# imironhead/ml_super_resolution

Measured on AMD Instinct MI355X. Metric: VDSR-20 training patches/sec (41x41, batch 256 per GPU); fwd HR megapixels/sec alongside, higher is better.
Workload: dtype f32; 1 GPU; BASELINE configs[2]: VDSR 20-layer 3x3x64 residual, RGB, batch 256x41x41 per GPU, fwd+bwd+TF-Adam, random-init weights; global_batch=256, patch=41, parallelism=dp1

## Files before the change

### include/srx.h

```cpp
#ifndef SRX_H_
#define SRX_H_

#include <stddef.h>
#include <stdint.h>

#ifdef __cplusplus
extern "C" {
#endif

typedef void* srx_stream_t;

typedef enum {
    SRX_OK = 0,
    SRX_ERR_BAD_ARG = -1,
    SRX_ERR_UNSUPPORTED = -2,
    SRX_ERR_WORKSPACE = -3,
    SRX_ERR_LAUNCH = -4,
    SRX_ERR_ALIGN = -5
} srx_status;

typedef enum { SRX_PAD_SAME = 0, SRX_PAD_VALID = 1 } srx_pad_mode;

typedef enum {
    SRX_ACT_NONE = 0,
// ... 33 lines not shown

int srx_set_chain_fixed(int on);

int srx_conv2d_precision_supported(const srx_conv_desc* d, int op);

size_t srx_conv2d_workspace_bytes(const srx_conv_desc* d, int op);

int srx_conv2d_fwd(const srx_conv_desc* d, const float* x, const float* w, const float* bias,
                   const float* skip, float* y, void* ws, size_t ws_bytes, srx_stream_t stream);

int srx_conv2d_bwd_data(const srx_conv_desc* d, const float* dpre, const float* w,
                        const float* x_in, int in_act, float* dx_out, void* ws, size_t ws_bytes,
                        srx_stream_t stream);

int srx_conv2d_bwd_data_acc(const srx_conv_desc* d, const float* dpre, const float* w, const float* dx_acc,
                            float* dx_out, void* ws, size_t ws_bytes, srx_stream_t stream);

int srx_conv2d_bwd_filter(const srx_conv_desc* d, const float* x, const float* dpre, float* dw,
                          float* dbias, const float* w_for_decay, float wd_scale, void* ws,
                          size_t ws_bytes, srx_stream_t stream);

int srx_conv2d_bwd_filter_partials(const srx_conv_desc* d, const float* x, const float* dpre, void* ws,
                                   size_t ws_bytes, int* n_partials, srx_stream_t stream);
int srx_conv2d_bwd_filter_reduce(const srx_conv_desc* d, const void* ws, int n_partials, float* dw,
                                 float* dbias, const float* w_for_decay, float wd_scale,
                                 srx_stream_t stream);

int srx_conv2d_bwd_filter_batch(const srx_conv_desc* d, int n_layers, const float* const* x, const float* const* dpre,
                                float* const* dw, float* const* dbias, const float* const* w_for_decay, float wd_scale,
                                void* ws, size_t ws_bytes, srx_stream_t stream);
size_t srx_conv2d_bwd_filter_batch_workspace_bytes(const srx_conv_desc* d, int n_layers);
int srx_conv2d_bwd_filter_batch_plan(const srx_conv_desc* d, int n_layers, int* wgs_per_layer, int* grid);
int srx_set_wgrad_batch(int on);

int srx_act_bwd(const float* dy, const float* y, float* dpre, size_t numel, int act,
                srx_stream_t stream);

int srx_depth_to_space(const float* in, float* out, int N, int H, int W, int C, int r,
                       srx_stream_t stream);

int srx_stream_copy(const void* in, void* out, size_t bytes, srx_stream_t stream);

int srx_espcn_forward(const float* x, const float* w1, const float* b1, const float* w2, const float* b2,
                      const float* w3, const float* b3, float* hr, int N, int H, int W, int r,
                      srx_stream_t stream);
int srx_espcn_forward_keep(const float* x, const float* w1, const float* b1, const float* w2, const float* b2,
                           const float* w3, const float* b3, float* t1, float* t2, float* y, int N, int H, int W, int r,
                           srx_stream_t stream);

int srx_srcnn_forward(const float* x, const float* w1, const float* b1, const float* w2, const float* b2,
                      const float* w3, const float* b3, float* y, int N, int H, int W, srx_stream_t stream);

int srx_space_to_depth(const float* in, float* out, int N, int H, int W, int C, int r,
                       srx_stream_t stream);

int srx_mse_fwd_bwd(const float* pred, const float* target, size_t numel, float inv_numel,
                    float* loss_out, int accumulate, float* dpred, void* scratch,
                    srx_stream_t stream);

int srx_l2_loss(const float* w, const float* mask, size_t numel, float scale, float* loss_out,
                int accumulate, void* scratch, srx_stream_t stream);

size_t srx_reduce_scratch_bytes(void);

int srx_adam_tf_step(float* w, const float* g, float* m, float* v, size_t numel, float lr,
                     float beta1, float beta2, float eps, int64_t t, float grad_scale,
// ... 287 lines not shown
```

### ml_super_resolution_amd/_lib.py

```python
import ctypes
import os

_HERE = os.path.dirname(os.path.abspath(__file__))
LIB_PATH = os.path.join(_HERE, 'libsrx.so')

SRX_OK = 0
PAD_SAME, PAD_VALID = 0, 1
ACT_NONE, ACT_RELU, ACT_TANH, ACT_LRELU, ACT_SIGMOID = 0, 1, 2, 3, 4
OP_FWD, OP_BWD_DATA, OP_BWD_FILTER = 0, 1, 2
PRECISION_FP32, PRECISION_BF16X3 = 0, 1
PRECISION_BY_NAME = {'highest': PRECISION_FP32, 'high': PRECISION_BF16X3}

ACT_BY_NAME = {None: ACT_NONE, 'none': ACT_NONE, 'relu': ACT_RELU, 'tanh': ACT_TANH,
               'lrelu': ACT_LRELU, 'leaky_relu': ACT_LRELU, 'sigmoid': ACT_SIGMOID}
PAD_BY_NAME = {'same': PAD_SAME, 'valid': PAD_VALID}

EXPORTS = [
    'srx_version', 'srx_last_error', 'srx_set_conv_path', 'srx_set_wgrad_path', 'srx_set_chain', 'srx_set_chain_fixed', 'srx_conv_chain', 'srx_conv_chain_supported', 'srx_conv2d_precision_supported', 'srx_conv2d_workspace_bytes', 'srx_conv2d_fwd',
    'srx_conv2d_bwd_data', 'srx_conv2d_bwd_filter', 'srx_conv2d_bwd_filter_partials', 'srx_conv2d_bwd_filter_reduce',
    'srx_conv2d_bwd_filter_batch', 'srx_conv2d_bwd_filter_batch_workspace_bytes', 'srx_conv2d_bwd_filter_batch_plan', 'srx_set_wgrad_batch', 'srx_act_bwd', 'srx_depth_to_space',
    'srx_space_to_depth', 'srx_stream_copy', 'srx_mse_fwd_bwd', 'srx_l2_loss', 'srx_reduce_scratch_bytes',
    'srx_adam_tf_step', 'srx_adam_tf_step_dev', 'srx_momentum_clip_step', 'srx_rownorm_loss_fwd_bwd', 'srx_psnr', 'srx_ssim', 'srx_ssim_scratch_bytes', 'srx_saturate_u8', 'srx_affine', 'srx_u8_to_unit_float', 'srx_gaussian_blur', 'srx_resize_bilinear',
    'srx_upsample_nearest', 'srx_upsample_nearest_bwd', 'srx_add_relu_grad',
    'srx_conv2d_bwd_data_acc', 'srx_conv3x3_blocked', 'srx_conv3x3_blocked_bwd_filter_workspace_bytes', 'srx_conv3x3_blocked_bwd_filter',
    'srx_conv3x3_blocked_ex', 'srx_conv3x3_blocked_bwd_filter_ex_workspace_bytes', 'srx_conv3x3_blocked_bwd_filter_ex',
    'srx_espcn_forward', 'srx_espcn_forward_keep', 'srx_debug_poison_lds', 'srx_srcnn_forward', 'srx_maxpool2x2', 'srx_maxpool2x2_bwd', 'srx_maxpool2x2_bwd_masked', 'srx_subsample2', 'srx_subsample2_bwd',
    'srx_channel_blocks_to_nhwc', 'srx_nhwc_to_channel_blocks', 'srx_channel_normalize', 'srx_channel_normalize_bwd',
    'srx_extract_patches16', 'srx_texture_gram', 'srx_texture_gram_bwd', 'srx_pil_resample_ksize', 'srx_pil_resample_coeffs', 'srx_resample_u8', 'srx_u8_to_pm1', 'srx_log_loss', 'srx_vgg_preprocess', 'srx_add_scaled', 'srx_resize_bicubic_tf', 'srx_column_sums', 'srx_gemm_workspace_bytes', 'srx_gemm',
    'srx_feature_mosaic_u8', 'srx_summary_panel_bytes', 'srx_summary_panel_range_bytes', 'srx_summary_panel_u8', 'srx_summary_panel_range',
    'srx_vdsr_patch_table_check', 'srx_vdsr_patch_pairs',
    'srx_espcn_patch_table_check', 'srx_espcn_patch_pairs',
    'srx_espcn_eval_table_check', 'srx_espcn_eval_tiles', 'srx_espcn_eval_pairs',
    'srx_vdsr_eval_table_check', 'srx_vdsr_eval_tiles', 'srx_vdsr_eval_footprint', 'srx_vdsr_eval_pairs',
    'srx_enet_pairs_table_words', 'srx_enet_pairs_tables', 'srx_enet_patch_table_check', 'srx_enet_patch_pairs',
    'srx_enet_eval_coeff_words', 'srx_enet_eval_coeffs', 'srx_enet_eval_table_check', 'srx_enet_eval_tiles', 'srx_enet_eval_footprint',
    'srx_enet_eval_pairs',
    'srx_image_scores_scratch_bytes', 'srx_image_scores_plan', 'srx_image_scores_lds_bytes', 'srx_image_scores',
    'srx_srcnn_pairs_band', 'srx_srcnn_pairs_lds_bytes', 'srx_srcnn_patch_table_check', 'srx_srcnn_patch_pairs',
    'srx_srcnn_eval_table_check', 'srx_srcnn_eval_tiles', 'srx_srcnn_eval_footprint', 'srx_srcnn_eval_pairs',
]


class SrxError(RuntimeError):
    pass


class ConvDesc(ctypes.Structure):
    _fields_ = [(n, ctypes.c_int32) for n in
                ('N', 'H', 'W', 'Cin', 'Cout', 'KH', 'KW', 'stride', 'pad_mode', 'act',
                 'post_add_relu', 'precision', 'subpixel_r')]


class PatchSrc(ctypes.Structure):
# ... 64 lines not shown
    global _lib
    if _lib is not None:
        return _lib
    if not os.path.exists(LIB_PATH):
        raise SrxError('libsrx.so not found at %s -- build it with `make -C %s` (or '
                       '__graft_entry__.build()); there is no CPU fallback' %
                       (LIB_PATH, os.path.join(_HERE, 'csrc')))
    import torch
    L = ctypes.CDLL(LIB_PATH)
    vp, sz, i, f = ctypes.c_void_p, ctypes.c_size_t, ctypes.c_int, ctypes.c_float
    dp = ctypes.POINTER(ConvDesc)
    L.srx_version.restype = ctypes.c_char_p
    L.srx_last_error.restype = ctypes.c_char_p
    L.srx_set_conv_path.argtypes = [i]
    L.srx_set_wgrad_path.argtypes = [i]
    L.srx_set_chain.argtypes = [i]
    L.srx_set_chain_fixed.argtypes = [i]
    L.srx_conv_chain_supported.argtypes = [dp, i, i]
    L.srx_conv_chain.argtypes = [dp, i, i, i, vp, vp, vp, vp, vp, vp]
    L.srx_conv2d_precision_supported.argtypes = [dp, i]
    L.srx_conv2d_workspace_bytes.argtypes = [dp, i]
    L.srx_conv2d_workspace_bytes.restype = sz
    L.srx_reduce_scratch_bytes.restype = sz
    L.srx_conv2d_fwd.argtypes = [dp, vp, vp, vp, vp, vp, vp, sz, vp]
    L.srx_conv2d_bwd_data.argtypes = [dp, vp, vp, vp, i, vp, vp, sz, vp]
    L.srx_conv2d_bwd_filter.argtypes = [dp, vp, vp, vp, vp, vp, f, vp, sz, vp]
    L.srx_conv2d_bwd_filter_partials.argtypes = [dp, vp, vp, vp, sz, ctypes.POINTER(ctypes.c_int), vp]
    L.srx_conv2d_bwd_filter_reduce.argtypes = [dp, vp, i, vp, vp, vp, f, vp]
    L.srx_conv2d_bwd_filter_batch.argtypes = [dp, i, vp, vp, vp, vp, vp, f, vp, sz, vp]
    L.srx_conv2d_bwd_filter_batch_workspace_bytes.argtypes = [dp, i]
    L.srx_conv2d_bwd_filter_batch_workspace_bytes.restype = sz
    L.srx_conv2d_bwd_filter_batch_plan.argtypes = [dp, i, ctypes.POINTER(ctypes.c_int), ctypes.POINTER(ctypes.c_int)]
    L.srx_set_wgrad_batch.argtypes = [i]
    L.srx_act_bwd.argtypes = [vp, vp, vp, sz, i, vp]
    L.srx_depth_to_space.argtypes = [vp, vp, i, i, i, i, i, vp]
    L.srx_space_to_depth.argtypes = [vp, vp, i, i, i, i, i, vp]
    L.srx_stream_copy.argtypes = [vp, vp, sz, vp]
    L.srx_mse_fwd_bwd.argtypes = [vp, vp, sz, f, vp, i, vp, vp, vp]
    L.srx_l2_loss.argtypes = [vp, vp, sz, f, vp, i, vp, vp]
    L.srx_adam_tf_step.argtypes = [vp, vp, vp, vp, sz, f, f, f, f, ctypes.c_int64, f, vp]
    L.srx_adam_tf_step_dev.argtypes = [vp, vp, vp, vp, sz, vp, f, f, f, f, vp]
    L.srx_momentum_clip_step.argtypes = [vp, vp, vp, sz, f, f, f, f, vp]
    L.srx_rownorm_loss_fwd_bwd.argtypes = [vp, vp, sz, sz, vp, vp, vp, vp]
    L.srx_psnr.argtypes = [vp, vp, vp, i, sz, f, vp]
    L.srx_ssim.argtypes = [vp, vp, vp, i, i, i, i, f, vp, vp]
    L.srx_ssim_scratch_bytes.argtypes = [i]
    L.srx_ssim_scratch_bytes.restype = sz
    sp, ip = ctypes.POINTER(ScoresDesc), ctypes.POINTER(ctypes.c_int)
    L.srx_image_scores_scratch_bytes.argtypes = [sp]
    L.srx_image_scores_scratch_bytes.restype = sz
    L.srx_image_scores_plan.argtypes = [sp, ip, ip, ip, ip]
    L.srx_image_scores_lds_bytes.argtypes = [sp]
    L.srx_image_scores_lds_bytes.restype = sz
    L.srx_image_scores.argtypes = [sp, vp, vp, vp, vp, vp]
    L.srx_saturate_u8.argtypes = [vp, vp, sz, vp]
    L.srx_feature_mosaic_u8.argtypes = [vp, vp, i, i, i, vp]
    L.srx_summary_panel_bytes.argtypes = [vp, i, i, i, i]
    L.srx_summary_panel_bytes.restype = sz
    L.srx_summary_panel_range_bytes.restype = sz
    L.srx_summary_panel_u8.argtypes = [vp, i, i, i, i, vp, vp, vp]
    L.srx_summary_panel_range.argtypes = [vp, i, i, i, i, vp, vp]
    L.srx_vdsr_patch_table_check.argtypes = [vp, i, i, sz]
    L.srx_vdsr_patch_pairs.argtypes = [vp, vp, i, i, vp, vp, vp]
    L.srx_espcn_patch_table_check.argtypes = [vp, i, i, i, sz]
    L.srx_espcn_patch_pairs.argtypes = [vp, vp, i, i, i, vp, vp, vp]
    L.srx_espcn_eval_table_check.argtypes = [vp, i, i, sz, sz]
# ... 82 lines not shown
```

### ml_super_resolution_amd/csrc/conv_narrow.hip

```cpp
#include "launchers.h"
namespace srx {
typedef float f32x3 __attribute__((ext_vector_type(3)));
typedef unsigned u32x3v __attribute__((ext_vector_type(3)));

template <int CTRL>
__device__ __forceinline__ float dpp_add(float v) {
    const int moved = __builtin_amdgcn_update_dpp(0, __float_as_int(v), CTRL, 0xf, 0xf, false);
    return v + __int_as_float(moved);
}

struct PixWalk {
    int n, oh, ow;
    __device__ __forceinline__ void init(unsigned p, int OH, int OW) {
        const unsigned t = p / (unsigned)OW;
        ow = (int)(p - t * (unsigned)OW);
        n = (int)(t / (unsigned)OH);
        oh = (int)(t - (unsigned)n * (unsigned)OH);
    }
    __device__ __forceinline__ void step16(int OH, int OW) { step(16, OH, OW); }
    __device__ __forceinline__ void step(int d, int OH, int OW) {
        ow += d;
        while (ow >= OW) {
            ow -= OW;
            oh += 1;
// ... 157 lines not shown
                idx = tc * CW + 4 * l + e;
            }
            part[idx] = r;
        } else {
            const int b = i - TAPS * 4 * CN;
            if constexpr (NOUT) {
                if (l == 0) part[wn + b] = r;
            } else {
                part[wn + 4 * l + b] = r;
            }
        }
    }
}

bool launch_wgrad_narrow(const ConvKey& k, const WgradArgs& a, int grid, hipStream_t s, hipError_t* err) {
    if (k.kh != 3 || k.kw != 3) return false;
    const bool nout = a.Cin == 64 && a.Cout == 3, nin = a.Cin == 3 && a.Cout == 64, nin32 = a.Cin == 3 && a.Cout == 32;
    if (!nout && !nin && !nin32) return false;
    const long total = (long)a.N * a.OH * a.OW;
    if (total >= (1L << 31) - 4096 || (long)a.N * a.H * a.W * 64 * 4 >= (1L << 31) - 4096 || total * 64 * 4 >= (1L << 31) - 4096)
        return false;
    const long ppi = nin32 ? 32 : 16;
    const int iters = (int)((total + ppi * grid - 1) / (ppi * grid));
    if (nout)
        hipLaunchKernelGGL((wgrad_narrow_kernel<3, 3, true>), dim3(grid), dim3(256), 0, s, a, total, iters);
    else if (nin)
        hipLaunchKernelGGL((wgrad_narrow_kernel<3, 3, false>), dim3(grid), dim3(256), 0, s, a, total, iters);
    else
        hipLaunchKernelGGL((wgrad_narrow_kernel<3, 3, false, 32>), dim3(grid), dim3(256), 0, s, a, total, iters);
    *err = hipGetLastError();
    return true;
}

bool launch_conv_narrow(const ConvKey& k, const ConvArgs& a, hipStream_t s, hipError_t* err) {
    if (k.wt || a.Cout != 3 || a.mask) return false;
    if ((long)a.N * a.H * a.W * a.Cin * 4 >= (1L << 31) - 4096) return false;
    const long total = (long)a.N * a.OH * a.OW;
    int iters = 16;
    while (iters > 1 && total / (16L * iters) < 2048) iters >>= 1;
    const long blocks = (total + 16L * iters - 1) / (16L * iters);
    if (total >= (1L << 31) - 4096) return false;
    if (k.kh == 3 && k.kw == 3 && a.Cin == 64) {
        hipLaunchKernelGGL((conv_narrow_kernel<3, 3, 64, 3>), dim3((unsigned)blocks), dim3(256), 0, s, a, total, iters);
    } else {
        return false;
    }
    *err = hipGetLastError();
    return true;
}
}
```

### ml_super_resolution_amd/csrc/launchers.h

```cpp
#pragma once
#include "conv_kernels.hip.h"
#include "lds_launch.h"

namespace srx {

struct ConvKey {
    int kh, kw, cinp, nch;
    bool wt;
};

bool launch_conv_k3c64(const ConvKey& k, const ConvArgs& a, int grid, size_t lds, hipStream_t s, hipError_t* err);
bool launch_conv_k3c32(const ConvKey& k, const ConvArgs& a, int grid, size_t lds, hipStream_t s, hipError_t* err);
bool launch_conv_c4(const ConvKey& k, const ConvArgs& a, int grid, size_t lds, hipStream_t s, hipError_t* err);
bool launch_conv_misc(const ConvKey& k, const ConvArgs& a, int grid, size_t lds, hipStream_t s, hipError_t* err);
bool launch_pipe_k3c64(const ConvKey& k, const ConvArgs& a, int grid, size_t lds, hipStream_t s, hipError_t* err);
bool launch_pipe_other(const ConvKey& k, const ConvArgs& a, int grid, size_t lds, hipStream_t s, hipError_t* err);
bool launch_wgrad_narrow(const ConvKey& k, const WgradArgs& a, int grid, hipStream_t s, hipError_t* err);
bool launch_conv_narrow(const ConvKey& k, const ConvArgs& a, hipStream_t s, hipError_t* err);
bool launch_conv_1x1(const ConvKey& k, const ConvArgs& a, long min_pixels, hipStream_t s, hipError_t* err);
bool launch_conv_rows3x3(const ConvKey& k, const ConvArgs& a, long min_pixels, hipStream_t s, hipError_t* err);
bool launch_conv_pack3(const ConvKey& k, const ConvArgs& a, long min_pixels, hipStream_t s, hipError_t* err);
bool launch_conv_kwrows(const ConvKey& k, const ConvArgs& a, long min_pixels, hipStream_t s, hipError_t* err);
bool launch_pipe_strip(const ConvKey& k, const ConvArgs& a, int grid, size_t lds, hipStream_t s, hipError_t* err);
bool launch_conv_generic(const ConvKey& k, const ConvArgs& a, int grid, size_t lds, hipStream_t s, hipError_t* err);
bool launch_wgrad(const ConvKey& k, const WgradArgs& a, int grid, size_t lds, hipStream_t s, hipError_t* err);
bool launch_wgrad_generic(const ConvKey& k, const WgradArgs& a, int grid, size_t lds, hipStream_t s, hipError_t* err);
bool launch_wgrad_lin(const ConvKey& k, const WgradArgs& a, int grid, size_t lds, hipStream_t s, hipError_t* err);
bool launch_wgrad_lin_pack3(const ConvKey& k, const WgradArgs& a, int grid, size_t lds, hipStream_t s, hipError_t* err);
bool launch_wgrad_lin_strip(const ConvKey& k, const WgradArgs& a, int grid, size_t lds, hipStream_t s, hipError_t* err);
bool launch_wgrad_pipe(const ConvKey& k, const WgradArgs& a, int grid, size_t lds, hipStream_t s, hipError_t* err);
bool launch_wgrad_kwcols(const ConvKey& k, const WgradArgs& a, int max_partials, long min_pixels, int* n_partials, hipStream_t s, hipError_t* err);
bool launch_wgrad_1x1(const ConvKey& k, const WgradArgs& a, int max_partials, int* n_partials, hipStream_t s, hipError_t* err);
bool launch_wgrad_rows_full(const ConvKey& k, const WgradArgs& a, int grid, size_t lds, hipStream_t s, hipError_t* err);
bool launch_wgrad_rows_strip(const ConvKey& k, const WgradArgs& a, int grid, size_t lds, hipStream_t s, hipError_t* err);
bool launch_wgrad_lin_pairs(const ConvKey& k, const WgradPairs& q, int grid, int pairs, bool strips, size_t lds, hipStream_t s, hipError_t* err);

__attribute__((weak)) hipError_t launch_conv_chain(bool wt, bool aux, bool fixed, const ConvArgs& a, const ChainPtrs& c, int grid, size_t lds, hipStream_t s);

__attribute__((weak)) hipError_t launch_wgrad_rows_batch(const WgradArgs& a, const WgradBatchPtrs& c, int wpl, int layers, size_t lds, hipStream_t s);
__attribute__((weak)) hipError_t launch_wgrad_batch_reduce(const float* part, int wpl, int layers, int stride, int wn, int cout,
                                                           const WgradBatchOut& o, float wd, hipStream_t s);

hipError_t launch_reduce_partials(const float* part, int G, int stride, int wn, int cout, float* dw, float* dbias,
                                  const float* w, float wd, hipStream_t s);
hipError_t launch_reduce_partials_pairs(const float* part, int G, int stride, int wn, int cout, float* dw, float* dbias,
                                        int pairs, int cob, hipStream_t s);

#define SRX_LAUNCH(...) launch_with_lds<__VA_ARGS__>(dim3(grid), dim3(256), lds, s, a)

#define SRX_CONV_CASE(KH, KW, CINP, NCH, WT, MINW)                                                        \
    if (k.kh == KH && k.kw == KW && k.cinp == CINP && k.nch == NCH && k.wt == WT) {                       \
        if (a.skip || a.mask)                                                                             \
            *err = SRX_LAUNCH(conv_mfma_kernel<KH, KW, CINP, NCH, WT, MINW, true>);                       \
        else                                                                                              \
            *err = SRX_LAUNCH(conv_mfma_kernel<KH, KW, CINP, NCH, WT, MINW, false>);                      \
        return true;                                                                                      \
    }
#define SRX_PIPE_CASE_FWD(KH, KW, CINP, NCH)                                                              \
    if (k.kh == KH && k.kw == KW && k.cinp == CINP && k.nch == NCH && !k.wt) {                            \
        if (a.skip)                                                                                       \
            *err = SRX_LAUNCH(conv_pipe_kernel<KH, KW, CINP, NCH, false, 2>);                             \
        else                                                                                              \
            *err = SRX_LAUNCH(conv_pipe_kernel<KH, KW, CINP, NCH, false, 0>);                             \
        return true;                                                                                      \
    }
#define SRX_PIPE_CASE_DGRAD(KH, KW, CINP, NCH)                                                            \
    if (k.kh == KH && k.kw == KW && k.cinp == CINP && k.nch == NCH && k.wt) {                             \
        if (a.mask)                                                                                       \
            *err = SRX_LAUNCH(conv_pipe_kernel<KH, KW, CINP, NCH, true, 1>);                              \
        else                                                                                              \
            *err = SRX_LAUNCH(conv_pipe_kernel<KH, KW, CINP, NCH, true, 0>);                              \
        return true;                                                                                      \
    }
#define SRX_PIPE_STRIP_CASE(KH, KW, CINP, NCH)                                                            \
// ... 50 lines not shown
```

### ml_super_resolution_amd/csrc/srx_api.hip

```cpp
#include <math.h>
#include <stdarg.h>
#include <atomic>
#include <stdio.h>
#include <stdlib.h>
#include <string.h>

#include "../../include/srx.h"
#include "elementwise.h"
#include "launchers.h"
#include "bf16x3.h"
#include "image_scores.h"

using namespace srx;

namespace {

thread_local char g_err[512] = "";

struct Knobs {
    int pipe_default, narrow, wgrad_lin, wgrad_pipe, wgrad_pipe_strip, wgrad_rows_full, wgrad_1x1, wgrad_pack3, kwrows_min_pixels, big_route_min_pixels, strip_d2s, conv_1x1_min_pixels, pack3_dgrad;
    int chain, chain_fixed, wgrad_batch;
    unsigned long long* trace;
    int dbg;
};
int env_int(const char* name, int dflt) { const char* e = getenv(name); return e ? atoi(e) : dflt; }
Knobs read_knobs() {
    Knobs k;
    k.pipe_default = env_int("SRX_PIPE", 1);
    k.narrow = env_int("SRX_NARROW", 1);
    k.wgrad_lin = env_int("SRX_WGRAD_LIN", 1);
    k.wgrad_pipe = env_int("SRX_WGRAD_PIPE", 1);
    k.wgrad_pipe_strip = env_int("SRX_WGRAD_PIPE_STRIP", 1);
    k.kwrows_min_pixels = env_int("SRX_KWROWS_MIN_PIXELS", 4096);
    k.big_route_min_pixels = env_int("SRX_BIG_ROUTE_MIN_PIXELS", 60000);
    k.conv_1x1_min_pixels = env_int("SRX_CONV_1X1_MIN_PIXELS", 100000);
    k.pack3_dgrad = env_int("SRX_PACK3_DGRAD", 1);
    k.strip_d2s = env_int("SRX_STRIP_D2S", 1);
    k.wgrad_rows_full = env_int("SRX_WGRAD_ROWS_FULL", 1);
    k.wgrad_1x1 = env_int("SRX_WGRAD_1X1", 1);
    k.wgrad_pack3 = env_int("SRX_WGRAD_PACK3", 1);
    k.chain = env_int("SRX_CHAIN", 1);
    k.chain_fixed = env_int("SRX_CHAIN_FIXED", 1);
    k.wgrad_batch = env_int("SRX_WGRAD_BATCH", 1);
    k.trace = nullptr;
    k.dbg = 0;
#ifdef SRX_TRACE
    { const char* tp = getenv("SRX_TRACE_PTR"); k.trace = tp ? (unsigned long long*)strtoull(tp, nullptr, 0) : nullptr; }
    k.dbg = env_int("SRX_DBG", 0);
#endif
    return k;
}
const Knobs& knobs() { static const Knobs k = read_knobs(); return k; }

template <int (*Dflt)()>
struct Toggle {
    std::atomic<int> v{-1};
    int get() const { const int x = v.load(std::memory_order_relaxed); return x < 0 ? Dflt() : x; }
    int set(int x) { const int old = v.exchange(x, std::memory_order_relaxed); return old < 0 ? Dflt() : old; }
};
inline int on_off(int on) { return on < 0 ? -1 : (on ? 1 : 0); }
inline int pipe_default() { return knobs().pipe_default; }
inline int chain_default() { return knobs().chain ? 1 : 0; }
inline int chain_fixed_default() { return knobs().chain_fixed ? 1 : 0; }
inline int wgrad_batch_default() { return knobs().wgrad_batch ? 1 : 0; }
inline int wgrad_path_default() { return !knobs().wgrad_lin ? 0 : ((knobs().wgrad_pipe || knobs().wgrad_pipe_strip) ? 2 : 1); }
Toggle<pipe_default> g_use_pipe;
Toggle<chain_default> g_chain;
Toggle<chain_fixed_default> g_chain_fixed;
Toggle<wgrad_batch_default> g_wgrad_batch;
Toggle<wgrad_path_default> g_wgrad_path;
int use_pipe() { return g_use_pipe.get(); }
int wgrad_path() { return g_wgrad_path.get(); }

int cu_count() {
    static std::atomic<int> cached[64];
    int dev = 0;
    if (hipGetDevice(&dev) != hipSuccess || dev < 0 || dev >= 64) { (void)hipGetLastError(); return 256; }
    int n = cached[dev].load(std::memory_order_relaxed);
    if (n > 0) return n;
    if (hipDeviceGetAttribute(&n, hipDeviceAttributeMultiprocessorCount, dev) != hipSuccess || n <= 0) {
        (void)hipGetLastError();
        n = 256;
    }
    if (n > 256) n = 256;
    cached[dev].store(n, std::memory_order_relaxed);
    return n;
}

int fail(int code, const char* fmt, ...) {
    va_list ap;
    va_start(ap, fmt);
    vsnprintf(g_err, sizeof(g_err), fmt, ap);
    va_end(ap);
    return code;
}
int launch_status(hipError_t err, const char* what) {
    return err == hipSuccess ? SRX_OK : fail(SRX_ERR_LAUNCH, "%s: %s", what, hipGetErrorString(err));
}
}
namespace srx {
int set_error(int code, const char* fmt, ...) {
    va_list ap;
// ... 613 lines not shown
    if (kn.narrow && !s2 && launch_wgrad_narrow(k, a, p.grid, s, &err)) return taken(p.grid);
    if (wgrad_rows_strip_ok(d, lp, wpath) && launch_wgrad_rows_strip(k, a, pgrid, 2 * lin_lds, s, &err)) return taken(pgrid);
    if (kn.wgrad_pack3 && lin_ok && lin_lds <= 80 * 1024 && d->Cin == 3 && launch_wgrad_lin_pack3(k, a, p.grid, lin_lds, s, &err)) return taken(p.grid);
    if (wgrad_lin_strip_ok(d, lp, wpath) && launch_wgrad_lin_strip(k, a, p.grid, lin_lds, s, &err)) return taken(p.grid);
    if (lin_ok && lin_lds <= 80 * 1024 && launch_wgrad_lin(k, a, p.grid, lin_lds, s, &err)) return taken(p.grid);
    if (launch_wgrad(k, a, p.grid, wg_lds, s, &err)) return taken(p.grid);
    if (wg_lds <= 80 * 1024 && launch_wgrad_generic(k, a, p.grid, wg_lds, s, &err)) return taken(p.grid);
    return fail(SRX_ERR_UNSUPPORTED, "no wgrad instance for %dx%d, Cin<=%d, Cout chunks %d%s", d->KH, d->KW, p.cinp,
                p.nch, s2 ? " at stride 2" : "");
}

int srx_conv2d_bwd_filter_reduce(const srx_conv_desc* d, const void* ws, int n_partials, float* dw, float* dbias,
                                 const float* w_for_decay, float wd_scale, srx_stream_t stream) {
    int rc = check_desc(d);
    if (rc) return rc;
    if (!ws || !dw) return fail(SRX_ERR_BAD_ARG, "null tensor pointer");
    if (d->precision == SRX_PRECISION_BF16X3 && (rc = bf16x3_supported(d, SRX_OP_BWD_FILTER)) != SRX_OK) return rc;
    if (n_partials <= 0 || n_partials > kMaxGridLimit) return fail(SRX_ERR_BAD_ARG, "bad partial count %d", n_partials);
    const size_t wn = (size_t)d->KH * d->KW * d->Cin * d->Cout;
    return launch_status(launch_reduce_partials((const float*)ws, n_partials, (int)part_stride(d), (int)wn, d->Cout, dw, dbias,
                                                w_for_decay, wd_scale, (hipStream_t)stream), "reduce launch failed");
}

int srx_conv2d_bwd_filter(const srx_conv_desc* d, const float* x, const float* dpre, float* dw, float* dbias,
                          const float* w_for_decay, float wd_scale, void* ws, size_t ws_bytes, srx_stream_t stream) {
    if (!dw) return fail(SRX_ERR_BAD_ARG, "null tensor pointer");
    int n = 0;
    const int rc = srx_conv2d_bwd_filter_partials(d, x, dpre, ws, ws_bytes, &n, stream);
    if (rc) return rc;
    return srx_conv2d_bwd_filter_reduce(d, ws, n, dw, dbias, w_for_decay, wd_scale, stream);
}

namespace {
int wgrad_batch_plan(const srx_conv_desc* d, int layers, WgradArgs* a, int* wpl, int* grid, size_t* lds) {
    int rc = check_desc(d);
    if (rc) return rc;
    if (!g_wgrad_batch.get()) return fail(SRX_ERR_UNSUPPORTED, "bwd_filter_batch: switched off (srx_set_wgrad_batch / SRX_WGRAD_BATCH)");
    if (!launch_wgrad_rows_batch || !launch_wgrad_batch_reduce) return fail(SRX_ERR_UNSUPPORTED, "bwd_filter_batch: this build has no batch kernels");
    if (layers < 2 || layers > kChainMax) return fail(SRX_ERR_UNSUPPORTED, "bwd_filter_batch: %d layers (2..%d)", layers, kChainMax);
    if (d->precision != SRX_PRECISION_FP32) return fail(SRX_ERR_UNSUPPORTED, "bwd_filter_batch: precision %d (exact fp32 only)", d->precision);
    if (d->KH != 3 || d->KW != 3 || d->Cin != 64 || d->Cout != 64 || d->stride != 1 || d->pad_mode != SRX_PAD_SAME)
        return fail(SRX_ERR_UNSUPPORTED, "bwd_filter_batch: only 3x3 64->64 stride-1 SAME layers");
    if (d->W != 41) return fail(SRX_ERR_UNSUPPORTED, "bwd_filter_batch: W %d (only 41-pixel rows: wgrad_rows_full_kernel's shape)", d->W);
    const int wpath = wgrad_path();
    if (!wgrad_rows_full_switches(wpath))
        return fail(SRX_ERR_UNSUPPORTED, "bwd_filter_batch: the filter-gradient path is not wgrad_rows_full_kernel's (srx_set_wgrad_path)");
    LayerPlan lp;
    if ((rc = plan_layer(d, SRX_OP_BWD_FILTER, true, true, &lp)) != SRX_OK) return rc;
    if (!wgrad_rows_full_ok(d, lp, wpath)) return fail(SRX_ERR_UNSUPPORTED, "bwd_filter_batch: the shape is not on wgrad_rows_full_kernel's route");
    const long rows = (long)d->N * lp.OH;
    long w = pipe_grid() / layers;
    if (w > rows) w = rows;
    if (w < 1) return fail(SRX_ERR_UNSUPPORTED, "bwd_filter_batch: %d layers on a grid of %d", layers, pipe_grid());
    *wpl = (int)w;
    *grid = pipe_grid();
    fill_wgrad_args(a, d, lp);
    *lds = set_wgrad_rows_full_tile(a);
    return SRX_OK;
}
}

int srx_set_wgrad_batch(int on) { return g_wgrad_batch.set(on_off(on)); }

int srx_conv2d_bwd_filter_batch_plan(const srx_conv_desc* d, int n_layers, int* wgs_per_layer, int* grid) {
    WgradArgs a;
    int wpl = 0, g = 0;
// ... 416 lines not shown
```

### ml_super_resolution_amd/engine.py

```python
import contextlib
import gc
import math
import os

import torch

from . import ops
from .param_pool import ParamPool


@contextlib.contextmanager
def capture_graph(g):
    gc.collect()
    was_enabled = gc.isenabled()
    gc.disable()
    try:
        with torch.cuda.graph(g):
            yield
    finally:
        if was_enabled:
            gc.enable()


class LayerSpec(object):
# ... 170 lines not shown
                if ops.bwd_filter_batch_plan(acts[i].shape, s.kernel_shape, j - i, s.padding)[0] > 0:
                    best = (i, j - 1)
            i = max(j, i + 1)
        return best

    def loss_and_backward(self, target, numel_global=None):
        if self._acts is None:
            raise RuntimeError('forward(keep=True) must run before loss_and_backward')
        acts = self._acts
        y = acts[-1]
        last = len(self.specs) - 1
        inv = 1.0 / (y.numel() if numel_global is None else numel_global)
        if self.loss_kind == 'rownorm':
            row_len = y.shape[1] * y.shape[2]
            dy = ops.rownorm_loss_fwd_bwd(y, target, row_len, self.loss, dpred=self._buf(('dy', 0), y.shape),
                                          norms=self._buf(('rownorms',), (y.numel() // row_len,)))
        else:
            dy = self._buf(('dy', 0), y.shape)
            ops.mse_fwd_bwd(y, target, self.loss, inv_numel=inv, accumulate=False, dpred=dy)
        if self.weight_decay:
            self.add_regulariser_loss()
        if self.specs[last].act is not None:
            dpre = ops.act_bwd(dy, y, self.specs[last].act, out=self._buf(('dpre_last',), y.shape))
        else:
            dpre = dy
        prec = self.layer_precision
        need = max(ops.bwd_filter_workspace_bytes(acts[i].shape, s.kernel_shape, s.padding, precision=prec[i])
                   for i, s in enumerate(self.specs))
        batch = self._wgrad_batch(acts)
        if batch is not None:
            b_lo, b_hi = batch
            need = max(need, ops.bwd_filter_batch_workspace_bytes(acts[b_lo].shape, self.specs[b_lo].kernel_shape, b_hi - b_lo + 1,
                                                                  self.specs[b_lo].padding))
        if self._ws is None or self._ws.numel() * 4 < need:
            self._step_graphs.clear()
            self._ws = torch.empty((need + 3) // 4, dtype=torch.float32, device=self.device)
        chain = self._dgrad_chain(acts)
        in_batch = lambda k: batch is not None and batch[0] <= k <= batch[1]
        dpres = {}

        def wgrad(i, dpre_i):
            s = self.specs[i]
            if not in_batch(i):
                ops.conv2d_bwd_filter(acts[i], dpre_i, s.kernel_shape, s.padding,
                                      w_for_decay=self.kernel(i) if self.weight_decay else None,
                                      wd_scale=self.weight_decay, dw=self.kernel(i, self.grads),
                                      dbias=self.bias(i, self.grads), workspace=self._ws, precision=prec[i])
                return
            dpres[i] = dpre_i
            if i == batch[0]:
                ks = list(range(batch[0], batch[1] + 1))
                ops.conv2d_bwd_filter_batch([acts[k] for k in ks], [dpres[k] for k in ks], [self.kernel(k, self.grads) for k in ks],
                                            [self.bias(k, self.grads) for k in ks],
                                            [self.kernel(k) for k in ks] if self.weight_decay else None, self.weight_decay,
                                            s.padding, workspace=self._ws)

        for i in range(last, -1, -1):
            s = self.specs[i]
            if chain is not None and chain[0] <= i <= chain[1]:
                lo, hi = chain
                if i == hi:
                    outs = [self._buf(('dpre_chain', k - 1), acts[k].shape) for k in range(hi, lo - 1, -1)]
                    ops.conv2d_bwd_data_chain([dpre] + outs[:-1], [self.kernel(k) for k in range(hi, lo - 1, -1)],
                                              [acts[k] for k in range(hi, lo - 1, -1)], outs, acts[hi].shape, s.padding,
                                              in_act=self.specs[hi - 1].act)
                    cdpres = {hi: dpre}
                    for k in range(hi, lo - 1, -1):
                        cdpres[k - 1] = outs[hi - k]
                wgrad(i, cdpres[i])
                if i == lo:
                    dpre = cdpres[lo - 1]
                continue
            wgrad(i, dpre)
            if i > 0:
                prev_act = self.specs[i - 1].act
                out = (self._buf(('dpre_chain', i - 1), acts[i].shape) if in_batch(i - 1)
                       else self._buf(('dx', i % 3, acts[i].shape[3]), acts[i].shape))
                dpre = ops.conv2d_bwd_data(dpre, self.kernel(i), acts[i].shape, s.padding,
                                           x_in=acts[i] if prev_act is not None else None, in_act=prev_act, out=out,
                                           precision=prec[i])
        if self.grad_hook is not None:
            self.grad_hook(self.grads)
        return self.loss

    def add_regulariser_loss(self):
        if self._decay_mask is None:
            self._decay_mask = torch.zeros_like(self.params)
            for i in range(len(self.specs)):
                self.kernel(i, self._decay_mask).fill_(1.0)
        ops.l2_loss(self.params, self.weight_decay, self.loss, accumulate=True, mask=self._decay_mask)

    def train_step_replay(self, x, target, lr, beta1=0.9, beta2=0.999, eps=1e-8, momentum=None, gradient_cap=0.01):
        def optimizer_launch():
            if momentum is None:
                self.adam_launch_dev(beta1, beta2, eps)
            else:
                ops.momentum_clip_step(self.params, self.grads, self.opt_m, lr, momentum, gradient_cap / lr)

        def eager(xx, tt):
            self.forward(xx, keep=True)
            self.loss_and_backward(tt)
            if momentum is None:
                self.adam_step_dev(lr, beta1, beta2, eps)
            else:
                self.momentum_clip_step(lr, momentum, gradient_cap)
            return self.loss
        if not self.use_step_graph or self.grad_hook is not None or self.device.type != 'cuda':
            return eager(x, target)
        if self.step_graph_max_pixels is not None and x.shape[0] * x.shape[1] * x.shape[2] > self.step_graph_max_pixels:
            return eager(x, target)
# ... 108 lines not shown
```

### ml_super_resolution_amd/ops.py

```python
import ctypes
import os

import numpy as np
import torch

from . import _lib
from ._lib import ACT_BY_NAME, PAD_BY_NAME, ConvDesc, check
from ._lib import lib as _load_lib

_POISON_LDS = os.environ.get('SRX_POISON_LDS', '0') == '1'


def lib():
    L = _load_lib()
    if _POISON_LDS and torch.cuda.is_available():
        L.srx_debug_poison_lds(_stream())
    return L



def _stream():
    return ctypes.c_void_p(torch.cuda.current_stream().cuda_stream)


# ... 177 lines not shown
    return wpl.value, grid.value


def bwd_filter_batch_workspace_bytes(x_shape, w_shape, n_layers, padding='same', stride=1, precision='highest'):
    d = conv_desc(x_shape, w_shape, padding, stride=stride, precision=precision)
    return _load_lib().srx_conv2d_bwd_filter_batch_workspace_bytes(ctypes.byref(d), int(n_layers))


def conv2d_bwd_filter_batch(xs, dpres, dws, dbiases=None, w_for_decay=None, wd_scale=0.0, padding='same', workspace=None,
                            stride=1, precision='highest'):
    L = len(xs)
    if not (len(dpres) == len(dws) == L) or (dbiases is not None and len(dbiases) != L) or (w_for_decay is not None and len(w_for_decay) != L):
        raise ValueError('conv2d_bwd_filter_batch: the per-layer lists differ in length')
    for l in range(L):
        _chk(xs[l], 'x'); _chk(dpres[l], 'dpre'); _chk(dws[l], 'dw')
        _chk(None if dbiases is None else dbiases[l], 'dbias'); _chk(None if w_for_decay is None else w_for_decay[l], 'w_for_decay')
    d = conv_desc(xs[0].shape, dws[0].shape, padding, stride=stride, precision=precision)
    for l in range(L):
        if tuple(xs[l].shape) != tuple(xs[0].shape) or tuple(dpres[l].shape) != tuple(out_shape(d)) or tuple(dws[l].shape) != tuple(dws[0].shape):
            raise ValueError('conv2d_bwd_filter_batch: layer %d does not have the shape of layer 0' % l)
    if workspace is None:
        need = _load_lib().srx_conv2d_bwd_filter_batch_workspace_bytes(ctypes.byref(d), L)
        workspace = torch.empty((max(need, 16) + 3) // 4, dtype=torch.float32, device=xs[0].device)
    _chk(workspace, 'workspace')
    check(lib().srx_conv2d_bwd_filter_batch(ctypes.byref(d), L, _ptr_array(xs), _ptr_array(dpres), _ptr_array(dws),
                                            None if dbiases is None else _ptr_array(dbiases),
                                            None if w_for_decay is None else _ptr_array(w_for_decay), float(wd_scale),
                                            _ptr(workspace), workspace.numel() * 4, _stream()), 'srx_conv2d_bwd_filter_batch')
    return dws, dbiases


def set_wgrad_batch(on):
    return lib().srx_set_wgrad_batch(int(on))


def act_bwd(dy, y, act, out=None):
    _chk(dy, 'dy'); _chk(y, 'y')
    out = out if out is not None else torch.empty_like(dy)
    check(lib().srx_act_bwd(_ptr(dy), _ptr(y), _ptr(out), dy.numel(), ACT_BY_NAME[act], _stream()), 'srx_act_bwd')
    return out


def depth_to_space(x, r, out=None):
    _chk(x, 'x')
    N, H, W, D = x.shape
    if D % (r * r):
        raise ValueError('depth %d not divisible by r*r=%d' % (D, r * r))
    C = D // (r * r)
    out = out if out is not None else torch.empty((N, H * r, W * r, C), dtype=torch.float32, device=x.device)
    check(lib().srx_depth_to_space(_ptr(x), _ptr(out), N, H, W, C, r, _stream()), 'srx_depth_to_space')
    return out


def espcn_forward(x, params, r, out=None):
    _chk(x, 'x')
    for k, b in params:
        _chk(k, 'kernel'); _chk(b, 'bias')
    (w1, b1), (w2, b2), (w3, b3) = params
    N, H, W, C = x.shape
    if C != 3 or tuple(w1.shape) != (5, 5, 3, 64) or tuple(w2.shape) != (3, 3, 64, 32) or tuple(w3.shape) != (3, 3, 32, 3 * r * r):
        raise ValueError('espcn_forward: shapes do not describe ESPCN 5-3-3 with scaling factor %d' % r)
    out = out if out is not None else torch.empty((N, H * r, W * r, 3), dtype=torch.float32, device=x.device)
    check(lib().srx_espcn_forward(_ptr(x), _ptr(w1), _ptr(b1), _ptr(w2), _ptr(b2), _ptr(w3), _ptr(b3), _ptr(out),
                                  N, H, W, int(r), _stream()), 'srx_espcn_forward')
    return out

# ... 1095 lines not shown
```

Baseline: 20310 patches/s.

## Fuse data and filter gradients for the final 64->3 conv layer

Adds a fused backward kernel for the last 3x3 64->3 conv. A single pass reads x and dpre once and computes the input gradient (with ReLU masking), the weight-gradient partials and the bias partials, followed by a separate reduce. It replaces separate wgrad and dgrad launches that each re-read the same tensors. The engine enables it by default when the layer fits the supported shape, which adds a new code path with its own workspace sizing.

```diff
diff --git a/include/srx.h b/include/srx.h
--- a/include/srx.h
+++ b/include/srx.h
@@ -89,6 +89,13 @@
 size_t srx_conv2d_bwd_filter_batch_workspace_bytes(const srx_conv_desc* d, int n_layers);
 int srx_conv2d_bwd_filter_batch_plan(const srx_conv_desc* d, int n_layers, int* wgs_per_layer, int* grid);
 int srx_set_wgrad_batch(int on);
+
+int srx_conv2d_bwd_out3(const srx_conv_desc* d, const float* x, const float* dpre, const float* w, int in_act, float* dx,
+                        float* dw, float* dbias, const float* w_for_decay, float wd_scale, void* ws, size_t ws_bytes,
+                        srx_stream_t stream);
+size_t srx_conv2d_bwd_out3_workspace_bytes(const srx_conv_desc* d);
+int srx_conv2d_bwd_out3_plan(const srx_conv_desc* d, int in_act, int* grid, int* iters);
+int srx_set_bwd_out3(int on);
 
 int srx_act_bwd(const float* dy, const float* y, float* dpre, size_t numel, int act,
                 srx_stream_t stream);
diff --git a/ml_super_resolution_amd/_lib.py b/ml_super_resolution_amd/_lib.py
--- a/ml_super_resolution_amd/_lib.py
+++ b/ml_super_resolution_amd/_lib.py
@@ -18,7 +18,8 @@
 EXPORTS = [
     'srx_version', 'srx_last_error', 'srx_set_conv_path', 'srx_set_wgrad_path', 'srx_set_chain', 'srx_set_chain_fixed', 'srx_conv_chain', 'srx_conv_chain_supported', 'srx_conv2d_precision_supported', 'srx_conv2d_workspace_bytes', 'srx_conv2d_fwd',
     'srx_conv2d_bwd_data', 'srx_conv2d_bwd_filter', 'srx_conv2d_bwd_filter_partials', 'srx_conv2d_bwd_filter_reduce',
-    'srx_conv2d_bwd_filter_batch', 'srx_conv2d_bwd_filter_batch_workspace_bytes', 'srx_conv2d_bwd_filter_batch_plan', 'srx_set_wgrad_batch', 'srx_act_bwd', 'srx_depth_to_space',
+    'srx_conv2d_bwd_filter_batch', 'srx_conv2d_bwd_filter_batch_workspace_bytes', 'srx_conv2d_bwd_filter_batch_plan', 'srx_set_wgrad_batch',
+    'srx_conv2d_bwd_out3', 'srx_conv2d_bwd_out3_workspace_bytes', 'srx_conv2d_bwd_out3_plan', 'srx_set_bwd_out3', 'srx_act_bwd', 'srx_depth_to_space',
     'srx_space_to_depth', 'srx_stream_copy', 'srx_mse_fwd_bwd', 'srx_l2_loss', 'srx_reduce_scratch_bytes',
     'srx_adam_tf_step', 'srx_adam_tf_step_dev', 'srx_momentum_clip_step', 'srx_rownorm_loss_fwd_bwd', 'srx_psnr', 'srx_ssim', 'srx_ssim_scratch_bytes', 'srx_saturate_u8', 'srx_affine', 'srx_u8_to_unit_float', 'srx_gaussian_blur', 'srx_resize_bilinear',
     'srx_upsample_nearest', 'srx_upsample_nearest_bwd', 'srx_add_relu_grad',
@@ -149,6 +150,11 @@
     L.srx_conv2d_bwd_filter_batch_workspace_bytes.restype = sz
     L.srx_conv2d_bwd_filter_batch_plan.argtypes = [dp, i, ctypes.POINTER(ctypes.c_int), ctypes.POINTER(ctypes.c_int)]
     L.srx_set_wgrad_batch.argtypes = [i]
+    L.srx_conv2d_bwd_out3.argtypes = [dp, vp, vp, vp, i, vp, vp, vp, vp, f, vp, sz, vp]
+    L.srx_conv2d_bwd_out3_workspace_bytes.argtypes = [dp]
+    L.srx_conv2d_bwd_out3_workspace_bytes.restype = sz
+    L.srx_conv2d_bwd_out3_plan.argtypes = [dp, i, ctypes.POINTER(ctypes.c_int), ctypes.POINTER(ctypes.c_int)]
+    L.srx_set_bwd_out3.argtypes = [i]
     L.srx_act_bwd.argtypes = [vp, vp, vp, sz, i, vp]
     L.srx_depth_to_space.argtypes = [vp, vp, i, i, i, i, i, vp]
     L.srx_space_to_depth.argtypes = [vp, vp, i, i, i, i, i, vp]
diff --git a/ml_super_resolution_amd/csrc/conv_narrow.hip b/ml_super_resolution_amd/csrc/conv_narrow.hip
--- a/ml_super_resolution_amd/csrc/conv_narrow.hip
+++ b/ml_super_resolution_amd/csrc/conv_narrow.hip
@@ -213,6 +213,110 @@
     return true;
 }
 
+__global__ __launch_bounds__(256, 2) void bwd_out3_kernel(const Out3Args a, long total_px, int iters) {
+    constexpr int TAPS = 9, CN = 3, CW = 64;
+    constexpr int NV = TAPS * 4 * CN + CN;
+    __shared__ float sm[4 * NV * 16];
+    const int c4 = threadIdx.x & 15;
+    const int sub = threadIdx.x >> 4;
+    const int wave = threadIdx.x >> 6;
+    for (int i = threadIdx.x; i < TAPS * CN * CW; i += 256) {
+        const int e = i & 3, l = (i >> 2) & 15, jc = i >> 6, c = jc % CN, j = jc / CN;
+        sm[i] = a.w[((TAPS - 1 - j) * CW + 4 * l + e) * CN + c];
+    }
+    __syncthreads();
+    f32x2 acc[TAPS * CN * 2];
+    float db[CN];
+#pragma unroll
+    for (int i = 0; i < TAPS * CN * 2; ++i) acc[i] = f32x2{0.0f, 0.0f};
+#pragma unroll
+    for (int c = 0; c < CN; ++c) db[c] = 0.0f;
+    const int xbytes = a.N * a.H * a.W * CW * 4;
+    const __amdgpu_buffer_rsrc_t xrs = __builtin_amdgcn_make_buffer_rsrc(const_cast<float*>(a.x), 0, xbytes, 0x00020000);
+    const __amdgpu_buffer_rsrc_t drs = __builtin_amdgcn_make_buffer_rsrc(const_cast<float*>(a.dpre), 0, a.N * a.H * a.W * CN * 4, 0x00020000);
+    const __amdgpu_buffer_rsrc_t yrs = __builtin_amdgcn_make_buffer_rsrc(a.dx, 0, xbytes, 0x00020000);
+    const unsigned p0 = blockIdx.x * (unsigned)iters * 16u + sub;
+    const auto wide_off = [&](unsigned p) { return p < (unsigned)total_px ? (int)((p * CW + 4 * c4) * 4) : kOobOffset; };
+    PixWalk q;
+    q.init(p0 < (unsigned)total_px ? p0 : 0u, a.H, a.W);
+    const bool nomask = !a.relu_mask;
+    f32x4 xr[3];
+    f32x3 dr[3][TAPS];
+    xr[0] = __builtin_bit_cast(f32x4, __builtin_amdgcn_raw_buffer_load_b128(xrs, wide_off(p0), 0, 0));
+    xr[1] = __builtin_bit_cast(f32x4, __builtin_amdgcn_raw_buffer_load_b128(xrs, wide_off(p0 + 16u), 0, 0));
+    {
+        int off[TAPS];
+        tap_offsets<3, 3>(off, q, p0 < (unsigned)total_px, a.H, a.W, 1, 1, CN * 4, 0);
+#pragma unroll
+        for (int j = 0; j < TAPS; ++j) dr[0][j] = __builtin_bit_cast(f32x3, __builtin_amdgcn_raw_buffer_load_b96(drs, off[j], 0, 0));
+        q.step16(a.H, a.W);
+    }
+    typedef const volatile __attribute__((address_space(3))) f32x4* LdsFilter;
+    const LdsFilter wl = (LdsFilter)sm + c4;
+    for (int it = 0; it < iters; it += 3) {
+#pragma unroll
+        for (int s = 0; s < 3; ++s) {
+            if (it + s >= iters) break;
+            const unsigned p = p0 + (unsigned)(it + s) * 16u;
+            xr[(s + 2) % 3] = __builtin_bit_cast(f32x4, __builtin_amdgcn_raw_buffer_load_b128(xrs, wide_off(p + 32u), 0, 0));
+            int off[TAPS];
+            tap_offsets<3, 3>(off, q, p + 16u < (unsigned)total_px, a.H, a.W, 1, 1, CN * 4, 0);
+#pragma unroll
+            for (int j = 0; j < TAPS; ++j)
+                dr[(s + 1) % 3][j] = __builtin_bit_cast(f32x3, __builtin_amdgcn_raw_buffer_load_b96(drs, off[j], 0, 0));
+            q.step16(a.H, a.W);
+            const f32x4 xv = xr[s];
+            const f32x2 xp[2] = {f32x2{xv[0], xv[1]}, f32x2{xv[2], xv[3]}};
+            f32x2 dxp[2] = {f32x2{0.0f, 0.0f}, f32x2{0.0f, 0.0f}};
+#pragma unroll
+            for (int j = 0; j < TAPS; ++j)
+#pragma unroll
+                for (int c = 0; c < CN; ++c) {
+                    const float d = dr[s][j][c];
+                    const f32x2 dd = {d, d};
+                    const f32x4 w4 = wl[(j * CN + c) * 16];
+#pragma unroll
+                    for (int h = 0; h < 2; ++h) {
+                        acc[(j * CN + c) * 2 + h] = __builtin_elementwise_fma(xp[h], dd, acc[(j * CN + c) * 2 + h]);
+                        dxp[h] = __builtin_elementwise_fma(f32x2{w4[2 * h], w4[2 * h + 1]}, dd, dxp[h]);
+                    }
+                }
+#pragma unroll
+            for (int c = 0; c < CN; ++c) db[c] += dr[s][TAPS / 2][c];
+            f32x4 dx = {dxp[0][0], dxp[0][1], dxp[1][0], dxp[1][1]};
+#pragma unroll
+            for (int e = 0; e < 4; ++e) dx[e] = (xv[e] > 0.0f || nomask) ? dx[e] : 0.0f * dx[e];
+            __builtin_amdgcn_raw_buffer_store_b128(__builtin_bit_cast(u32x4v, dx), yrs, wide_off(p), 0, 0);
+        }
+    }
+    __syncthreads();
+#pragma unroll
+    for (int i = 0; i < NV; ++i) {
+        float r = i < NV - CN ? acc[i >> 1][i & 1] : db[i < NV - CN ? 0 : i - (NV - CN)];
+        r += __shfl_xor(r, 16);
+        r += __shfl_xor(r, 32);
+        if ((sub & 3) == 0) sm[(wave * NV + i) * 16 + c4] = r;
+    }
+    __syncthreads();
+    float* part = a.part + (size_t)blockIdx.x * a.part_stride;
+    for (int t = threadIdx.x; t < NV * 16; t += 256) {
+        const int i = t >> 4, l = t & 15;
+        const float r = (sm[(0 * NV + i) * 16 + l] + sm[(1 * NV + i) * 16 + l]) + (sm[(2 * NV + i) * 16 + l] + sm[(3 * NV + i) * 16 + l]);
+        if (i < NV - CN) {
+            const int e = i & 3, jc = i >> 2, c = jc % CN, j = jc / CN;
+            part[((TAPS - 1 - j) * CW + 4 * l + e) * CN + c] = r;
+        } else if (l == 0) {
+            part[TAPS * CW * CN + i - (NV - CN)] = r;
+        }
+    }
+}
+
+hipError_t launch_bwd_out3(const Out3Args& a, int grid, int iters, hipStream_t s) {
+    const long total = (long)a.N * a.H * a.W;
+    hipLaunchKernelGGL(bwd_out3_kernel, dim3(grid), dim3(256), 0, s, a, total, iters);
+    return hipGetLastError();
+}
+
 bool launch_conv_narrow(const ConvKey& k, const ConvArgs& a, hipStream_t s, hipError_t* err) {
     if (k.wt || a.Cout != 3 || a.mask) return false;
     if ((long)a.N * a.H * a.W * a.Cin * 4 >= (1L << 31) - 4096) return false;
diff --git a/ml_super_resolution_amd/csrc/launchers.h b/ml_super_resolution_amd/csrc/launchers.h
--- a/ml_super_resolution_amd/csrc/launchers.h
+++ b/ml_super_resolution_amd/csrc/launchers.h
@@ -40,6 +40,18 @@
 __attribute__((weak)) hipError_t launch_wgrad_rows_batch(const WgradArgs& a, const WgradBatchPtrs& c, int wpl, int layers, size_t lds, hipStream_t s);
 __attribute__((weak)) hipError_t launch_wgrad_batch_reduce(const float* part, int wpl, int layers, int stride, int wn, int cout,
                                                            const WgradBatchOut& o, float wd, hipStream_t s);
+
+struct Out3Args {
+    const float* x;
+    const float* dpre;
+    const float* w;
+    float* dx;
+    float* part;
+    int part_stride;
+    int N, H, W;
+    int relu_mask;
+};
+__attribute__((weak)) hipError_t launch_bwd_out3(const Out3Args& a, int grid, int iters, hipStream_t s);
 
 hipError_t launch_reduce_partials(const float* part, int G, int stride, int wn, int cout, float* dw, float* dbias,
                                   const float* w, float wd, hipStream_t s);
diff --git a/ml_super_resolution_amd/csrc/srx_api.hip b/ml_super_resolution_amd/csrc/srx_api.hip
--- a/ml_super_resolution_amd/csrc/srx_api.hip
+++ b/ml_super_resolution_amd/csrc/srx_api.hip
@@ -19,7 +19,7 @@
 
 struct Knobs {
     int pipe_default, narrow, wgrad_lin, wgrad_pipe, wgrad_pipe_strip, wgrad_rows_full, wgrad_1x1, wgrad_pack3, kwrows_min_pixels, big_route_min_pixels, strip_d2s, conv_1x1_min_pixels, pack3_dgrad;
-    int chain, chain_fixed, wgrad_batch;
+    int chain, chain_fixed, wgrad_batch, bwd_out3;
     unsigned long long* trace;
     int dbg;
 };
@@ -42,6 +42,7 @@
     k.chain = env_int("SRX_CHAIN", 1);
     k.chain_fixed = env_int("SRX_CHAIN_FIXED", 1);
     k.wgrad_batch = env_int("SRX_WGRAD_BATCH", 1);
+    k.bwd_out3 = env_int("SRX_BWD_OUT3", 1);
     k.trace = nullptr;
     k.dbg = 0;
 #ifdef SRX_TRACE
@@ -63,11 +64,13 @@
 inline int chain_default() { return knobs().chain ? 1 : 0; }
 inline int chain_fixed_default() { return knobs().chain_fixed ? 1 : 0; }
 inline int wgrad_batch_default() { return knobs().wgrad_batch ? 1 : 0; }
+inline int bwd_out3_default() { return (knobs().narrow && knobs().bwd_out3) ? 1 : 0; }
 inline int wgrad_path_default() { return !knobs().wgrad_lin ? 0 : ((knobs().wgrad_pipe || knobs().wgrad_pipe_strip) ? 2 : 1); }
 Toggle<pipe_default> g_use_pipe;
 Toggle<chain_default> g_chain;
 Toggle<chain_fixed_default> g_chain_fixed;
 Toggle<wgrad_batch_default> g_wgrad_batch;
+Toggle<bwd_out3_default> g_bwd_out3;
 Toggle<wgrad_path_default> g_wgrad_path;
 int use_pipe() { return g_use_pipe.get(); }
 int wgrad_path() { return g_wgrad_path.get(); }
@@ -747,6 +750,66 @@
 }
 
 namespace {
+int bwd_out3_plan(const srx_conv_desc* d, int in_act, int* grid, int* iters) {
+    int rc = check_desc(d);
+    if (rc) return rc;
+    if (!g_bwd_out3.get()) return fail(SRX_ERR_UNSUPPORTED, "bwd_out3: switched off (srx_set_bwd_out3 / SRX_BWD_OUT3 / SRX_NARROW)");
+    if (!launch_bwd_out3) return fail(SRX_ERR_UNSUPPORTED, "bwd_out3: this build has no bwd_out3 kernel");
+    if (d->precision != SRX_PRECISION_FP32) return fail(SRX_ERR_UNSUPPORTED, "bwd_out3: precision %d (exact fp32 only)", d->precision);
+    if (d->KH != 3 || d->KW != 3 || d->Cin != 64 || d->Cout != 3 || d->stride != 1 || d->pad_mode != SRX_PAD_SAME)
+        return fail(SRX_ERR_UNSUPPORTED, "bwd_out3: only 3x3 64->3 stride-1 SAME layers");
+    if (in_act != SRX_ACT_NONE && in_act != SRX_ACT_RELU) return fail(SRX_ERR_UNSUPPORTED, "bwd_out3: in_act %d (none / ReLU)", in_act);
+    const long total = (long)d->N * d->H * d->W;
+    if (total >= (1L << 31) - 4096 || total * 64 * 4 >= (1L << 31) - 4096)
+        return fail(SRX_ERR_UNSUPPORTED, "bwd_out3: the input tensor is beyond 31-bit byte offsets");
+    long g = (total + 15) / 16;
+    if (g > max_grid()) g = max_grid();
+    *grid = (int)g;
+    *iters = (int)((total + 16 * g - 1) / (16 * g));
+    return SRX_OK;
+}
+}
+
+int srx_set_bwd_out3(int on) { return g_bwd_out3.set(on_off(on)); }
+
+int srx_conv2d_bwd_out3_plan(const srx_conv_desc* d, int in_act, int* grid, int* iters) {
+    int g = 0, it = 0;
+    const int rc = bwd_out3_plan(d, in_act, &g, &it);
+    if (rc) { g = 0; it = 0; }
+    if (grid) *grid = g;
+    if (iters) *iters = it;
+    return rc;
+}
+
+size_t srx_conv2d_bwd_out3_workspace_bytes(const srx_conv_desc* d) {
+    int g = 0, it = 0;
+    if (bwd_out3_plan(d, SRX_ACT_NONE, &g, &it) != SRX_OK) return 0;
+    return partials_bytes(d, (size_t)g);
+}
+
+int srx_conv2d_bwd_out3(const srx_conv_desc* d, const float* x, const float* dpre, const float* w, int in_act, float* dx, float* dw,
+                        float* dbias, const float* w_for_decay, float wd_scale, void* ws, size_t ws_bytes, srx_stream_t stream) {
+    int grid = 0, iters = 0;
+    int rc = bwd_out3_plan(d, in_act, &grid, &iters);
+    if (rc) return rc;
+    if (!x || !dpre || !w || !dx || !dw) return fail(SRX_ERR_BAD_ARG, "null tensor pointer");
+    const auto aligned4 = [](const void* p) { return (reinterpret_cast<uintptr_t>(p) & 3u) == 0; };
+    if (!aligned16(x) || !aligned16(dpre) || !aligned16(w) || !aligned16(dx) || !aligned16(ws) || !aligned4(dw) || !aligned4(dbias) ||
+        !aligned4(w_for_decay))
+        return fail(SRX_ERR_UNSUPPORTED, "bwd_out3: x, dpre, w, dx and the workspace must be 16-byte aligned (dw, dbias, w_for_decay: 4)");
+    if (dx == x || dx == dpre) return fail(SRX_ERR_BAD_ARG, "bwd_out3: dx aliases an operand");
+    const size_t need = partials_bytes(d, (size_t)grid);
+    if (!ws || ws_bytes < need) return fail(SRX_ERR_WORKSPACE, "bwd_out3 needs %zu workspace bytes, got %zu", need, ws_bytes);
+    Out3Args a;
+    memset(&a, 0, sizeof(a));
+    a.x = x; a.dpre = dpre; a.w = w; a.dx = dx; a.part = (float*)ws; a.part_stride = (int)part_stride(d);
+    a.N = d->N; a.H = d->H; a.W = d->W; a.relu_mask = in_act == SRX_ACT_RELU;
+    if ((rc = launch_status(launch_bwd_out3(a, grid, iters, (hipStream_t)stream), "bwd_out3 launch failed")) != SRX_OK) return rc;
+    return launch_status(launch_reduce_partials((const float*)ws, grid, a.part_stride, 9 * 64 * 3, 3, dw, dbias, w_for_decay, wd_scale,
+                                                (hipStream_t)stream), "reduce launch failed");
+}
+
+namespace {
 int wgrad_batch_plan(const srx_conv_desc* d, int layers, WgradArgs* a, int* wpl, int* grid, size_t* lds) {
     int rc = check_desc(d);
     if (rc) return rc;
diff --git a/ml_super_resolution_amd/engine.py b/ml_super_resolution_amd/engine.py
--- a/ml_super_resolution_amd/engine.py
+++ b/ml_super_resolution_amd/engine.py
@@ -226,6 +226,12 @@
             b_lo, b_hi = batch
             need = max(need, ops.bwd_filter_batch_workspace_bytes(acts[b_lo].shape, self.specs[b_lo].kernel_shape, b_hi - b_lo + 1,
                                                                   self.specs[b_lo].padding))
+        fused_last = (last > 0 and prec[last] == 'highest' and self.specs[last - 1].act in (None, 'relu') and
+                      not (batch is not None and batch[0] <= last <= batch[1]) and
+                      ops.bwd_out3_plan(acts[last].shape, self.specs[last].kernel_shape, self.specs[last].padding,
+                                        in_act=self.specs[last - 1].act)[0] > 0)
+        if fused_last:
+            need = max(need, ops.bwd_out3_workspace_bytes(acts[last].shape, self.specs[last].kernel_shape, self.specs[last].padding))
         if self._ws is None or self._ws.numel() * 4 < need:
             self._step_graphs.clear()
             self._ws = torch.empty((need + 3) // 4, dtype=torch.float32, device=self.device)
@@ -265,11 +271,18 @@
                 if i == lo:
                     dpre = cdpres[lo - 1]
                 continue
-            wgrad(i, dpre)
+            if not (fused_last and i == last):
+                wgrad(i, dpre)
             if i > 0:
                 prev_act = self.specs[i - 1].act
                 out = (self._buf(('dpre_chain', i - 1), acts[i].shape) if in_batch(i - 1)
                        else self._buf(('dx', i % 3, acts[i].shape[3]), acts[i].shape))
+                if fused_last and i == last:
+                    dpre = ops.conv2d_bwd_out3(acts[i], dpre, self.kernel(i), s.padding, in_act=prev_act, dx=out,
+                                               dw=self.kernel(i, self.grads), dbias=self.bias(i, self.grads),
+                                               w_for_decay=self.kernel(i) if self.weight_decay else None,
+                                               wd_scale=self.weight_decay, workspace=self._ws)[0]
+                    continue
                 dpre = ops.conv2d_bwd_data(dpre, self.kernel(i), acts[i].shape, s.padding,
                                            x_in=acts[i] if prev_act is not None else None, in_act=prev_act, out=out,
                                            precision=prec[i])
diff --git a/ml_super_resolution_amd/ops.py b/ml_super_resolution_amd/ops.py
--- a/ml_super_resolution_amd/ops.py
+++ b/ml_super_resolution_amd/ops.py
@@ -233,6 +233,45 @@
 
 def set_wgrad_batch(on):
     return lib().srx_set_wgrad_batch(int(on))
+
+
+def bwd_out3_plan(x_shape, w_shape, padding='same', in_act=None, stride=1, precision='highest'):
+    d = conv_desc(x_shape, w_shape, padding, stride=stride, precision=precision)
+    grid, iters = ctypes.c_int(0), ctypes.c_int(0)
+    _load_lib().srx_conv2d_bwd_out3_plan(ctypes.byref(d), ACT_BY_NAME[in_act], ctypes.byref(grid), ctypes.byref(iters))
+    return grid.value, iters.value
+
+
+def bwd_out3_workspace_bytes(x_shape, w_shape, padding='same', stride=1, precision='highest'):
+    d = conv_desc(x_shape, w_shape, padding, stride=stride, precision=precision)
+    return _load_lib().srx_conv2d_bwd_out3_workspace_bytes(ctypes.byref(d))
+
+
+def conv2d_bwd_out3(x, dpre, w, padding='same', in_act=None, dx=None, dw=None, dbias=None, want_dbias=True, w_for_decay=None,
+                    wd_scale=0.0, workspace=None, stride=1, precision='highest'):
+    for t, n in ((x, 'x'), (dpre, 'dpre'), (w, 'w'), (w_for_decay, 'w_for_decay'), (dx, 'dx'), (dw, 'dw'), (dbias, 'dbias')):
+        _chk(t, n)
+    d = conv_desc(x.shape, w.shape, padding, stride=stride, precision=precision)
+    if tuple(dpre.shape) != tuple(out_shape(d)):
+        raise ValueError('dpre has shape %s, the layer output is %s' % (tuple(dpre.shape), tuple(out_shape(d))))
+    if dx is None:
+        dx = torch.empty(tuple(x.shape), dtype=torch.float32, device=x.device)
+    if dw is None:
+        dw = torch.empty(tuple(w.shape), dtype=torch.float32, device=x.device)
+    if dbias is None and want_dbias:
+        dbias = torch.empty((w.shape[3],), dtype=torch.float32, device=x.device)
+    if workspace is None:
+        need = _load_lib().srx_conv2d_bwd_out3_workspace_bytes(ctypes.byref(d))
+        workspace = torch.empty((max(need, 16) + 3) // 4, dtype=torch.float32, device=x.device)
+    _chk(workspace, 'workspace')
+    check(lib().srx_conv2d_bwd_out3(ctypes.byref(d), _ptr(x), _ptr(dpre), _ptr(w), ACT_BY_NAME[in_act], _ptr(dx), _ptr(dw),
+                                    _ptr(dbias), _ptr(w_for_decay), float(wd_scale), _ptr(workspace), workspace.numel() * 4,
+                                    _stream()), 'srx_conv2d_bwd_out3')
+    return dx, dw, dbias
+
+
+def set_bwd_out3(on):
+    return lib().srx_set_bwd_out3(int(on))
 
 
 def act_bwd(dy, y, act, out=None):
```

Measured after the change: 20310 patches/s (median of 3 runs). No clear change (+0.0%).
